# Quake4/WavPackDecoder

Hardware: AMD Instinct MI355X
Metric: Msamples/sec decoded (node) + HBM GB/s, batched 44.1kHz/16-bit stereo blocks (higher is better)
Workload: dtype int32; 1 GPU; C2: 1024-block batch, 16-bit stereo 'fast' {17,17}, joint stereo, 44.1 kHz; slices_rank0=1, blocks_rank0=1024, frames_rank0=22579200, frames_total=22579200, parallelism=file-shard x1, no collectives

## Files before the change

wavpackdecoder_amd/csrc/wv_lane.h:

```cpp
#pragma once
#include <hip/hip_runtime.h>

#include "wv_wave2.h"

namespace wvg {
namespace lane {

constexpr uint32_t ST_REDO = 1u << 15;
constexpr int RU = 32;
constexpr int GF = 8;
constexpr int NLD = 4;
constexpr int LPAIRS = 2;

__device__ __forceinline__ int32_t aw(int32_t w, int32_t s) {
    return (int32_t)(((int64_t)w * (int64_t)s + 512) >> 10);
}

template <int T, int U, bool MONO>
__device__ __forceinline__ void lp_frame(int32_t &wA, int32_t &wB, const int32_t dl, int32_t *hA, int32_t *hB, int32_t &L,
                                         int32_t &R) {
    using namespace wvf;
    static_assert(!MONO || T > 0, "mono lists have positive terms only");
    if constexpr (T == 17 || T == 18) {
        const int32_t sa = T == 17 ? sub32(mul32(2, hA[0]), hA[1]) : (sub32(mul32(3, hA[0]), hA[1]) >> 1);
// ... 579 lines not shown
            } else {
                s.zacc = lgamma(s, ring, rbase);
                if (s.zacc > 0u) {
                    s.m[0][0] = s.m[0][1] = s.m[0][2] = 0;
                    s.m[1][0] = s.m[1][1] = s.m[1][2] = 0;
                    zskip = true;
                }
            }
        }
    }
    const uint64_t zm = lmask(zskip);
    const uint64_t hzm = h0m0 | zm;
    if constexpr (HY) {
        s.slow[C] = zskip ? lhy_decay(s.slow[C]) : s.slow[C];
        if constexpr (C == 0) lhy_errlim(s, ring, !zskip);
    }
    const uint32_t lo = (uint32_t)s.win;
    uint32_t raw = (uint32_t)__builtin_ctz(~lo | 0x10000u);
    uint32_t p = raw + 1u;
    const uint64_t escm = lmask(raw >= 16u) & ~hzm;
    if (__builtin_expect(escm != 0ull, 0)) {
        if (__builtin_amdgcn_inverse_ballot_w64(escm)) {
            if (lo & 0x10000u) s.pmax = 17u;
            lskip(s, 17u);
            lrefill(s, ring, rbase);
            raw = lgamma(s, ring, rbase) + 16u;
            if (raw >= (1u << 24)) s.pmax = 17u;
            p = 0u;
        }
    }
    p = vselm(hzm, 0u, p);
    lskip(s, p);
    lrefill(s, ring, rbase);
    const uint32_t ones = vselm(hzm, 0u, addc(raw >> 1, h1m0));
    const uint64_t b0m = lmask((raw & 1u) != 0u);
    s.h1 = lbit(~hzm & b0m) ? 1u : 0u;
    s.keep = lbit(~hzm & ~b0m) ? 0u : ~0u;
    const int32_t m0 = s.m[C][0], m1 = s.m[C][1], m2 = s.m[C][2];
    const uint32_t a0 = (uint32_t)(m0 >> 4), a1 = (uint32_t)(m1 >> 4), a2 = (uint32_t)(m2 >> 4);
    const uint64_t o0 = lmask(ones == 0u), o1 = lmask(ones == 1u), o2 = lmask(ones == 2u), ob = o0 | o1;
    const uint32_t mc = vselm(o0, a0, vselm(o1, a1, a2));
    const uint32_t low1 = a0 + 1u;
    const uint32_t low2 = (ones > 2u ? ones - 2u : 0u) * (a2 + 1u) + low1 + a1 + 1u;
    const uint32_t low = vselm(o0, 0u, vselm(o1, low1, low2));
    s.m[C][0] = add32(m0, mul32((int32_t)(add3((uint32_t)m0, 128u, (uint32_t)csel<-2, 0>(o0))) >> 7, csel<-2, 5>(o0)));
    s.m[C][1] = add32(m1, mul32((int32_t)(add3((uint32_t)m1, 64u, (uint32_t)csel<-2, 0>(o1))) >> 6,
                                vselmi(o0, 0, csel<-2, 5>(o1))));
    s.m[C][2] = add32(m2, mul32((int32_t)(add3((uint32_t)m2, 32u, (uint32_t)csel<-2, 0>(o2))) >> 5,
                                vselmi(ob, 0, csel<-2, 5>(o2))));
    const uint32_t x = (uint32_t)s.win;
    uint32_t mid, used, lo_f = 0u, n_f = 1u;
    if constexpr (HY) {
        lhy_code<HY>(x, low, mc, s.el[C], mid, used, s.bad, lo_f, n_f);
        s.slack = min(s.slack, 31 - (int32_t)used);
    } else {
        const uint32_t z = (uint32_t)__builtin_clz(mc | 1u);
        const uint32_t ones_z = 0xFFFFFFFFu >> z;
        const uint32_t ex = ones_z - mc;
        const uint32_t nbt = z ^ 31u;
        const uint32_t v = x & (ones_z >> 1);
        const uint64_t bigm = lmask(v >= ex);
        const uint32_t code = vselm(bigm, 2u * v + __builtin_amdgcn_ubfe(x, nbt, 1) - ex, v);
        used = addc(nbt, bigm);
        mid = low + code;
    }
    const int32_t sg = __builtin_amdgcn_sbfe((int32_t)x, used, 1);
    lskip(s, vselm(zm, 0u, used + 1u));
    LW w;
    w.v = (int32_t)vselm(zm, 0u, mid ^ (uint32_t)sg);
    w.x = vselm(zm, 0u, x);
    w.low = vselm(zm, 0u, low);
    w.mc = vselm(zm, 0u, mc);
    w.clo = vselm(zm, 0u, mid);
    w.cn = 1u;
    if constexpr (HY == 2) {
        const bool inexact = !zskip && s.el[C] != 0;
        w.clo = inexact ? lo_f : w.clo;
        w.cn = inexact ? n_f : 1u;
    }
    if constexpr (HY) s.slow[C] = zskip ? s.slow[C] : lhy_slow(s.slow[C], mid, ring);
    lrefill(s, ring, rbase);
    return w;
}

template <int C>
__device__ __forceinline__ LW lword_fast(LState &s, const uint8_t *ring, uint32_t rbase) {
    using namespace wvf;
    const uint32_t zx = (((uint32_t)(s.m[0][0] | s.m[1][0])) & ~1u) | (s.keep + 1u) | s.h1;
    const uint32_t zrv = zx == 0u ? 1u : 0u;
    const uint32_t zdec = min(s.zacc, zrv);
    s.zacc -= zdec;
    const uint32_t zsk = min(s.zacc, zdec);
    const uint32_t lo = (uint32_t)s.win;
    const uint32_t raw = (uint32_t)__builtin_ctz(~lo | 0x10000u);
    const uint32_t keep = s.keep & (zsk - 1u);
    const uint32_t p = (raw + 1u) & keep;
    s.rare |= ((p + 15u) >> 5) | (zrv & (zdec ^ 1u));
    const uint32_t ones = ((raw >> 1) + s.h1) & keep;
    const uint32_t nh1 = raw & 1u & keep;
    s.h1 = nh1;
    s.keep = (uint32_t)__builtin_amdgcn_sbfe((int32_t)(nh1 | ~keep), 0, 1);
    s.win >>= p;
    s.nb -= (int32_t)p;
    const int32_t m0 = s.m[C][0], m1 = s.m[C][1], m2 = s.m[C][2];
    const uint32_t a0 = (uint32_t)(m0 >> 4), a1 = (uint32_t)(m1 >> 4), a2 = (uint32_t)(m2 >> 4);
    const bool o0 = ones == 0u, o1 = ones == 1u, o2 = ones == 2u, ob = ones < 2u;
    const uint32_t mc = o0 ? a0 : (o1 ? a1 : a2);
    const uint32_t low1 = a0 + 1u;
    const uint32_t low2 = __umul24(ones > 2u ? ones - 2u : 0u, a2 + 1u) + low1 + a1 + 1u;
    const uint32_t low = o0 ? 0u : (o1 ? low1 : low2);
    s.m[C][0] = mad24((add32(m0, o0 ? 126 : 128)) >> 7, o0 ? -2 : 5, m0);
    s.m[C][1] = mad24((add32(m1, o1 ? 62 : 64)) >> 6, o0 ? 0 : (o1 ? -2 : 5), m1);
    s.m[C][2] = mad24((add32(m2, o2 ? 30 : 32)) >> 5, ob ? 0 : (o2 ? -2 : 5), m2);
    const uint32_t x = (uint32_t)s.win;
    const uint32_t z = (uint32_t)__builtin_clz(mc | 1u);
    const uint32_t ones_z = 0xFFFFFFFFu >> z;
    const uint32_t ex = ones_z - mc;
    const uint32_t nbt = z ^ 31u;
    const uint32_t v = x & (ones_z >> 1);
    const bool big = v >= ex;
    const uint32_t code = big ? 2u * v + __builtin_amdgcn_ubfe(x, nbt, 1) - ex : v;
    const uint32_t used = nbt + (big ? 1u : 0u);
    const uint32_t mid = low + code;
    const int32_t sg = __builtin_amdgcn_sbfe((int32_t)x, used, 1);
    const uint32_t len = (used + 1u) & (zsk - 1u);
    s.win >>= len;
    s.nb -= (int32_t)len;
    s.slack = min(s.slack, s.nb);
    LW w;
    w.v = (int32_t)((mid ^ (uint32_t)sg) & (zsk - 1u));
    w.x = x & (zsk - 1u);
    w.low = low & (zsk - 1u);
    w.mc = mc & (zsk - 1u);
    w.clo = 0u;
    w.cn = 1u;
    lrefill(s, ring, rbase);
    return w;
}

template <bool NONNEG = true>
__device__ __forceinline__ void lmerge(LState &s, const uint8_t *ring) {
    const uint32_t mg = (uint32_t)((s.nb - 33) >> 31);
    uint32_t sh = (uint32_t)s.nb;
    if constexpr (NONNEG) __builtin_assume(sh < 64u);
    else sh &= 63u;
    s.win |= (uint64_t)(s.nxt & mg) << sh;
    s.nb = mad24((int32_t)mg, -32, s.nb);
    s.ra = ring_step(s.ra, mg);
    s.nxt = *(const uint32_t *)(ring + s.ra);
}
#ifndef WV_LANE_SPEC
#define WV_LANE_SPEC 0
#endif
template <int C, bool SPLIT, int HY = false, bool W32 = false>
__device__ __forceinline__ LW lword_nz(LState &s, const uint8_t *ring, uint32_t rbase) {
    static_assert(!HY || SPLIT, "a hybrid word's bisection bits follow a refill");
    using namespace wvf;
    constexpr bool SPEC = WV_LANE_SPEC && !SPLIT && !HY && !W32;
    const uint32_t lo = (uint32_t)s.win, hi = (uint32_t)(s.win >> 32);
    const uint32_t raw0 = SPEC ? s.r0 : (uint32_t)__builtin_ctz(~lo | 0x10000u);
    uint32_t ehi = 0u;
    if constexpr (SPEC) {
        const uint32_t sft = (uint32_t)(s.nb - 32) & 63u;
        ehi = hi | (uint32_t)((uint64_t)s.nxt << sft);
    }
    s.rmax = max(s.rmax, raw0);
    const uint32_t raw = raw0 & s.keep;
    const uint32_t ones = (raw >> 1) + s.h1;
    const uint32_t q = raw - s.keep;
    s.h1 = raw & 1u;
    s.keep = (uint32_t)__builtin_amdgcn_sbfe((int32_t)(raw | ~s.keep), 0, 1);
    if constexpr (HY && C == 0) lhy_errlim(s, ring, true);
    const int32_t m0 = s.m[C][0], m1 = s.m[C][1], m2 = s.m[C][2];
    const uint32_t a0 = (uint32_t)(m0 >> 4), a1 = (uint32_t)(m1 >> 4), a2 = (uint32_t)(m2 >> 4);
    const bool o0 = ones == 0u, o1 = ones == 1u;
    const uint32_t mc = o0 ? a0 : (o1 ? a1 : a2);
    const uint32_t l3 = (W32 ? (ones > 2u ? ones - 2u : 0u) * (a2 + 1u) : mul_u24(ones > 2u ? ones - 2u : 0u, a2 + 1u)) +
                        a1 + 1u;
    const uint32_t low = vselm(lmask(o0), 0u, add3(a0, 1u, vselm(lmask(o1), 0u, l3)));
    const uint32_t k4 = min(ones, 3u) << 2;
    const int32_t d0 = (int32_t)add3((uint32_t)m0, 128u, (uint32_t)__builtin_amdgcn_sbfe(0x000E, k4, 4)) >> 7;
    const int32_t d1 = (int32_t)add3((uint32_t)m1, 64u, (uint32_t)__builtin_amdgcn_sbfe(0x00E0, k4, 4)) >> 6;
    const int32_t d2 = (int32_t)add3((uint32_t)m2, 32u, (uint32_t)__builtin_amdgcn_sbfe(0x0E00, k4, 4)) >> 5;
    const int32_t x0 = __builtin_amdgcn_sbfe(0x555E, k4, 4), x1 = __builtin_amdgcn_sbfe(0x55E0, k4, 4);
    const int32_t x2 = __builtin_amdgcn_sbfe(0x5E00, k4, 4);
    if constexpr (W32) {
        s.m[C][0] = wvf::add32(m0, wvf::mul32(d0, x0));
        s.m[C][1] = wvf::add32(m1, wvf::mul32(d1, x1));
        s.m[C][2] = wvf::add32(m2, wvf::mul32(d2, x2));
    } else {
        s.m[C][0] = mad24(d0, x0, m0);
        s.m[C][1] = mad24(d1, x1, m1);
        s.m[C][2] = mad24(d2, x2, m2);
    }
    uint32_t x;
    if constexpr (SPLIT) {
        __builtin_assume(q < 64u);
        s.win >>= q;
        s.nb -= (int32_t)q;
        s.slack = min(s.slack, s.nb);
        lmerge<false>(s, ring);
        x = (uint32_t)s.win;
    } else {
        x = __builtin_amdgcn_alignbit(hi, lo, q);
    }
    uint32_t mid, used, lo_f = 0u, n_f = 1u;
    if constexpr (HY) {
        lhy_code<HY>(x, low, mc, s.el[C], mid, used, s.bad, lo_f, n_f);
        s.slack = min(s.slack, 31 - (int32_t)used);
    } else {
        const uint32_t z = (uint32_t)__builtin_clz(mc | 1u);
        const uint32_t ex = (0xFFFFFFFFu >> z) - mc;
        const uint32_t nbt = z ^ 31u;
        const uint32_t v = __builtin_amdgcn_ubfe(x, 0, nbt);
        const bool big = v >= ex;
        const uint32_t t = v + __builtin_amdgcn_ubfe(x, nbt, 1) - ex;
        mid = add3(low, v, big ? t : 0u);
        used = nbt + (big ? 1u : 0u);
    }
    const int32_t sg = __builtin_amdgcn_sbfe((int32_t)x, used, 1);
    const uint32_t tot = SPLIT ? used + 1u : add3(q, used, 1u);
    __builtin_assume(tot < 64u);
    if constexpr (SPEC) s.r0 = (uint32_t)__builtin_ctz(~(uint32_t)((((uint64_t)ehi << 32) | lo) >> tot) | 0x10000u);
    s.win >>= tot;
    s.nb -= (int32_t)tot;
    s.slack = min(s.slack, s.nb);
    if constexpr (!SPLIT) lmerge(s, ring);
    if constexpr (HY) s.slow[C] = lhy_slow(s.slow[C], mid, ring);
#ifdef WV_LANE_WORD_BARRIER
    __builtin_amdgcn_sched_barrier(WV_LANE_WORD_BARRIER);
#endif
    uint32_t clo = mid, cn = 1u;
    if constexpr (HY == 2) {
        clo = s.el[C] != 0 ? lo_f : mid;
        cn = s.el[C] != 0 ? n_f : 1u;
    }
    return LW{x, low, mc, (int32_t)(mid ^ (uint32_t)sg), clo, cn};
}

constexpr int RF = 24;
static_assert(RF % GF == 0, "a group's frames never wrap the frame ring");
constexpr uint32_t LSPIN = 1u << 24;

struct LShared {
    int4 rq[RF * 64];
    int2 rm[RF * 64];
    uint32_t pflag[64];
    uint32_t produced, consumed, abort;
    uint32_t hop_out[3], hop_in[3];
    uint32_t rbh[2][64];
};

__device__ __forceinline__ uint32_t rpos(const LState &s) { return s.rp + (((s.ra0 - s.ra) & RSLOT) >> 8); }

template <int HY>
__device__ __forceinline__ uint32_t pverdict(const LState &s, uint32_t u0) {
    const uint32_t r = s.bad | (s.pmax >= 17u ? 16u : 0u) | (s.slack < 0 ? 32u : 0u) | (rpos(s) >= u0 * 4u ? 64u : 0u);
    return 0x80000000u | r | ((s.bad0 ? s.bad0 : r) << 8);
}

enum { WK_CHECKED = 0, WK_FAST = 1, WK_NORUN = 2, WK_NORUN_SPLIT = 3, WK_NORUN_SPLIT32 = 4 };
template <int K, int C, int HY>
__device__ __forceinline__ LW lword_k(LState &s, const uint8_t *ring, uint32_t rb) {
    if constexpr (K == WK_NORUN) return lword_nz<C, false, false>(s, ring, rb);
    else if constexpr (K == WK_NORUN_SPLIT) return lword_nz<C, true, HY>(s, ring, rb);
    else if constexpr (K == WK_NORUN_SPLIT32) return lword_nz<C, true, HY, true>(s, ring, rb);
    else if constexpr (K == WK_FAST) return lword_fast<C>(s, ring, rb);
    else return lword<C, HY>(s, ring, rb);
}
template <int U, bool FULL, int FAST, bool MONO, int HY, bool CODES>
__device__ __forceinline__ void pframe(LState &s, const uint8_t *ring, uint32_t rb, LShared &sh, uint32_t lane,
                                       uint32_t g0, uint32_t nfr, uint32_t u0, uint32_t &pfin) {
    const uint32_t t = g0 + U;
    const uint32_t slot = (((g0 % (uint32_t)RF) + U) << 6) + lane;
    const LW w0 = lword_k<FAST, 0, HY>(s, ring, rb);
    LW w1 = {0u, 0u, 0u, 0, 0u, 1u};
    if constexpr (!MONO) w1 = lword_k<FAST, 1, HY>(s, ring, rb);
    if constexpr (CODES) {
        sh.rq[slot] = make_int4((int32_t)w0.x, (int32_t)w0.low, (int32_t)w1.x, (int32_t)w1.low);
        sh.rm[slot] = make_int2((int32_t)w0.mc, (int32_t)w1.mc);
    } else {
        sh.rm[slot] = make_int2(w0.v, w1.v);
        if constexpr (HY == 2)
            sh.rq[slot] = make_int4((int32_t)w0.clo, (int32_t)w0.cn, (int32_t)w1.clo, (int32_t)w1.cn);
    }
    if (!FULL && t + 1u == nfr) pfin = pverdict<HY>(s, u0);
}
template <bool FULL, int FAST, bool MONO, int HY, bool CODES>
__device__ __forceinline__ void pgroup(LState &s, const uint8_t *ring, uint32_t rb, LShared &sh, uint32_t lane,
                                       uint32_t g0, uint32_t nfr, uint32_t u0, uint32_t &pfin) {
    pframe<0, FULL, FAST, MONO, HY, CODES>(s, ring, rb, sh, lane, g0, nfr, u0, pfin);
    pframe<1, FULL, FAST, MONO, HY, CODES>(s, ring, rb, sh, lane, g0, nfr, u0, pfin);
    pframe<2, FULL, FAST, MONO, HY, CODES>(s, ring, rb, sh, lane, g0, nfr, u0, pfin);
    pframe<3, FULL, FAST, MONO, HY, CODES>(s, ring, rb, sh, lane, g0, nfr, u0, pfin);
    pframe<4, FULL, FAST, MONO, HY, CODES>(s, ring, rb, sh, lane, g0, nfr, u0, pfin);
    pframe<5, FULL, FAST, MONO, HY, CODES>(s, ring, rb, sh, lane, g0, nfr, u0, pfin);
    pframe<6, FULL, FAST, MONO, HY, CODES>(s, ring, rb, sh, lane, g0, nfr, u0, pfin);
    pframe<7, FULL, FAST, MONO, HY, CODES>(s, ring, rb, sh, lane, g0, nfr, u0, pfin);
}
#ifndef WV_LANE_COUNTERS
#define WV_LANE_COUNTERS 0
#endif
#define LCNT(x)                                 \
    do {                                        \
        if constexpr (WV_LANE_COUNTERS != 0) x; \
    } while (0)
struct LCount {
    uint32_t groups, bulk, norun, split, fast, checked, replay;
    uint64_t wait_consumed, wait_loads;
    uint64_t words, stage;
};
template <bool FULL, bool MONO, int HY, bool CODES>
__device__ __forceinline__ void pgroup_try(LState &s, const uint8_t *ring, uint32_t rb, LShared &sh, uint32_t lane,
                                           uint32_t g0, uint32_t nfr, uint32_t u0, uint32_t &pfin, uint32_t mm,
                                           LCount &cnt) {
    LCNT(cnt.groups++);
    const uint32_t livem = (uint32_t)((int32_t)(g0 - nfr) >> 31);
    s.slack = 0;
    constexpr uint32_t WPG = MONO ? GF : 2 * GF;
    const uint32_t notrun = (((uint32_t)(s.m[0][0] | s.m[1][0])) & ~1u) | ~s.keep | s.h1 | (s.zacc <= WPG ? 1u : 0u);
    if (lmask((notrun & livem) != 0u) == 0ull) {
#pragma unroll
        for (int u = 0; u < GF; u++) {
            const uint32_t slot = (((g0 % (uint32_t)RF) + u) << 6) + lane;
            if constexpr (CODES) sh.rq[slot] = make_int4(0, 0, 0, 0);
            if constexpr (HY == 2) sh.rq[slot] = make_int4(0, 1, 0, 1);
            sh.rm[slot] = make_int2(0, 0);
            if constexpr (HY) {
                s.slow[0] = lhy_decay(s.slow[0]);
                if constexpr (!MONO) s.slow[1] = lhy_decay(s.slow[1]);
            }
        }
        s.zacc -= WPG;
        if (!FULL && livem && nfr <= g0 + GF) pfin = pverdict<HY>(s, u0);
        LCNT(cnt.bulk++);
        return;
    }
    const uint32_t mml = mm & livem;
    const bool m26 = lmask(mml >= (1u << 26)) != 0ull;
    const uint32_t runnable = ((uint32_t)(max(s.m[0][0], s.m[1][0]) - (2 + 2 * GF)) >> 31) | min(s.zacc, 1u);
#ifndef WV_LANE_HY_PATH
#define WV_LANE_HY_PATH 0
#endif
    const bool allnr = lmask((runnable & livem) != 0u) == 0ull &&
                       !(HY && ((WV_LANE_HY_PATH == 1 && m26) || WV_LANE_HY_PATH == 2));
    if (__builtin_expect(m26 && !allnr, 0)) {
        pgroup<FULL, WK_CHECKED, MONO, HY, CODES>(s, ring, rb, sh, lane, g0, nfr, u0, pfin);
        s.bad |= s.slack < 0 ? 32u : 0u;
        LCNT(cnt.checked++);
        return;
    }
    const LState s0 = s;
    const uint32_t pfin0 = pfin;
    if (allnr) {
        s.rmax = 0u;
        if (__builtin_expect(m26, 0)) {
            pgroup<FULL, WK_NORUN_SPLIT32, MONO, HY, CODES>(s, ring, rb, sh, lane, g0, nfr, u0, pfin);
            lmerge<false>(s, ring);
            LCNT(cnt.split++);
        } else if (!HY && lmask(mml >= (1u << 17)) == 0ull) {
            if constexpr (WV_LANE_SPEC) s.r0 = (uint32_t)__builtin_ctz(~(uint32_t)s.win | 0x10000u);
            pgroup<FULL, WK_NORUN, MONO, HY, CODES>(s, ring, rb, sh, lane, g0, nfr, u0, pfin);
            LCNT(cnt.norun++);
        } else {
            pgroup<FULL, WK_NORUN_SPLIT, MONO, HY, CODES>(s, ring, rb, sh, lane, g0, nfr, u0, pfin);
            lmerge<false>(s, ring);
            LCNT(cnt.split++);
        }
        s.rare = s.rmax >> 4;
    } else if constexpr (HY) {
        s.slack = 0;
        pgroup<FULL, WK_CHECKED, MONO, HY, CODES>(s, ring, rb, sh, lane, g0, nfr, u0, pfin);
        s.bad |= s.slack < 0 ? 32u : 0u;
        LCNT(cnt.checked++);
        return;
    } else {
        s.rare = 0u;
        pgroup<FULL, WK_FAST, MONO, HY, CODES>(s, ring, rb, sh, lane, g0, nfr, u0, pfin);
        LCNT(cnt.fast++);
    }
    if (__builtin_expect(lmask(((s.rare | ((uint32_t)s.slack >> 31)) & livem) != 0u) != 0ull, 0)) {
        s = s0;
        pfin = pfin0;
        s.slack = 0;
        pgroup<FULL, WK_CHECKED, MONO, HY, CODES>(s, ring, rb, sh, lane, g0, nfr, u0, pfin);
        s.bad |= s.slack < 0 ? 32u : 0u;
        LCNT(cnt.replay++);
    }
}

struct LEnd {
    uint32_t *st;
    int32_t ml;
    bool check;
    int32_t crc;
    const uint32_t *pflag;
    uint32_t lane;
};
__device__ __forceinline__ void lane_finish(uint32_t rbad, const LEnd &e, int32_t mx, int32_t mn, uint32_t crc) {
    const uint32_t pf = e.pflag[e.lane];
    const uint32_t bad = (rbad | (pf & 0xFFu) | (mx > e.ml || mn < -e.ml ? 8u : 0u));
    uint32_t st = 0;
    if (e.check) {
        st |= ST_CRC_CHECKED;
        if ((int32_t)crc != e.crc) st |= ST_CRC_ERROR;
    }
    *e.st = bad ? (ST_REDO | (bad << 16) | (((pf >> 8) & 0xFFu) << 24)) : st;
}

__device__ __forceinline__ void st2(int32_t *p, int2 v) {
    p[0] = v.x;
    p[1] = v.y;
}

template <int HY>
__device__ __forceinline__ int32_t lfix(int32_t x, uint32_t sh, const Fixup &fx) {
    if constexpr (HY) return fixup_tail(fx, x);
    else return (int32_t)((uint32_t)x << sh);
}
__device__ __forceinline__ int32_t rdecode(uint32_t x, uint32_t low, uint32_t mc) {
    const uint32_t z = (uint32_t)__builtin_clz(mc | 1u);
    const uint32_t ex = (0xFFFFFFFFu >> z) - mc;
    const uint32_t nbt = z ^ 31u;
    const uint32_t v = __builtin_amdgcn_ubfe(x, 0, nbt);
    const bool big = v >= ex;
    const uint32_t t = v + __builtin_amdgcn_ubfe(x, nbt, 1) - ex;
    const uint32_t used = nbt + (big ? 1u : 0u);
    const int32_t sg = __builtin_amdgcn_sbfe((int32_t)x, used, 1);
    return (int32_t)(add3(low, v, big ? t : 0u) ^ (uint32_t)sg);
}
template <int U, bool MONO, bool CODES>
__device__ __forceinline__ void rin(const LShared &shr, uint32_t lane, uint32_t g0, int32_t &L, int32_t &R) {
    const uint32_t slot = (((g0 % (uint32_t)RF) + U) << 6) + lane;
    const int2 r = shr.rm[slot];
    if constexpr (CODES) {
        const int4 q = shr.rq[slot];
        L = rdecode((uint32_t)q.x, (uint32_t)q.y, (uint32_t)r.x);
        R = MONO ? 0 : rdecode((uint32_t)q.z, (uint32_t)q.w, (uint32_t)r.y);
    } else {
        L = r.x;
        R = r.y;
    }
}
template <int U, bool FULL, bool MONO, int HY>
__device__ __forceinline__ void rout(int32_t L, int32_t R, uint32_t g0, uint32_t nfr, bool joint, int32_t &mx,
                                     int32_t &mn, uint32_t &crc, uint32_t sh, int32_t *o, uint32_t rbad, const LEnd &e,
                                     bool fst, const Fixup &fx, const CWin &cw) {
    const uint32_t t = g0 + U;
    if constexpr (MONO) {
        mx = max(mx, L);
        mn = min(mn, L);
        crc = crc * 3u + (uint32_t)L;
        const int32_t v = lfix<HY>(L, sh, fx);
        const bool st = FULL ? nfr != 0u : t < nfr;
        if (st) {
            if (fst) st2(o + 2u * t, make_int2(v, v));
            else o[t] = v;
        }
        if (!FULL && t + 1u == nfr) lane_finish(rbad | (HY == 2 && (cw.used > cw.end || cw.ovf) ? 1u : 0u), e, mx, mn, crc);
        return;
    }
    if (joint) {
        R = wvf::sub32(R, L >> 1);
        L = wvf::add32(L, R);
    }
    mx = max(mx, max(L, R));
    mn = min(mn, min(L, R));
    crc = crc * 9u + (uint32_t)L * 3u + (uint32_t)R;
    int2 v;
    v.x = lfix<HY>(L, sh, fx);
    v.y = lfix<HY>(R, sh, fx);
    if (FULL) {
        if (nfr) st2(o + 2u * t, v);
    } else {
        if (t < nfr) st2(o + 2u * t, v);
        if (t + 1u == nfr) lane_finish(rbad | (HY == 2 && (cw.used > cw.end || cw.ovf) ? 1u : 0u), e, mx, mn, crc);
    }
}
template <int U, bool FULL, bool MONO, int HY, bool CODES, int... Ts>
__device__ __forceinline__ void rframe(LChain<Ts...> &ch, const LShared &shr, uint32_t lane, uint32_t g0, uint32_t nfr,
                                       bool joint, int32_t &mx, int32_t &mn, uint32_t &crc, uint32_t sh, int32_t *o,
                                       uint32_t rbad, const LEnd &e, bool fst, const Fixup &fx, CWin &cw) {
    const uint32_t t = g0 + U;
    int32_t L, R;
    rin<U, MONO, CODES>(shr, lane, g0, L, R);
    if constexpr (HY == 2) {
        const int4 q = shr.rq[(((g0 % (uint32_t)RF) + U) << 6) + lane];
        int32_t cL = 0, cR = 0;
        if (FULL || t < nfr) {
            cL = cwin_corr(cw, L, (uint32_t)q.x, (uint32_t)q.y);
            cR = cwin_corr(cw, R, (uint32_t)q.z, (uint32_t)q.w);
        }
        ch.template frame_wvc<U, MONO>(L, R, cL, cR);
        L = wvf::add32(L, cL);
        R = wvf::add32(R, cR);
    } else {
        ch.template frame<U, MONO>(L, R);
    }
    rout<U, FULL, MONO, HY>(L, R, g0, nfr, joint, mx, mn, crc, sh, o, rbad, e, fst, fx, cw);
}
template <bool FULL, bool MONO, bool CODES, int NS, int HY = 0>
__device__ __forceinline__ void rgroup_rt(RChain<NS> &ch, const LShared &shr, uint32_t lane, uint32_t g0, uint32_t nfr,
                                          bool joint, int32_t &mx, int32_t &mn, uint32_t &crc, uint32_t sh, int32_t *o,
                                          uint32_t rbad, const LEnd &e, bool fst, const Fixup &fx, const CWin &cw) {
    int32_t L[GF], R[GF];
    rin<0, MONO, CODES>(shr, lane, g0, L[0], R[0]);
    rin<1, MONO, CODES>(shr, lane, g0, L[1], R[1]);
    rin<2, MONO, CODES>(shr, lane, g0, L[2], R[2]);
    rin<3, MONO, CODES>(shr, lane, g0, L[3], R[3]);
    rin<4, MONO, CODES>(shr, lane, g0, L[4], R[4]);
    rin<5, MONO, CODES>(shr, lane, g0, L[5], R[5]);
    rin<6, MONO, CODES>(shr, lane, g0, L[6], R[6]);
    rin<7, MONO, CODES>(shr, lane, g0, L[7], R[7]);
    ch.template group<MONO>(L, R);
    rout<0, FULL, MONO, HY>(L[0], R[0], g0, nfr, joint, mx, mn, crc, sh, o, rbad, e, fst, fx, cw);
    rout<1, FULL, MONO, HY>(L[1], R[1], g0, nfr, joint, mx, mn, crc, sh, o, rbad, e, fst, fx, cw);
    rout<2, FULL, MONO, HY>(L[2], R[2], g0, nfr, joint, mx, mn, crc, sh, o, rbad, e, fst, fx, cw);
    rout<3, FULL, MONO, HY>(L[3], R[3], g0, nfr, joint, mx, mn, crc, sh, o, rbad, e, fst, fx, cw);
    rout<4, FULL, MONO, HY>(L[4], R[4], g0, nfr, joint, mx, mn, crc, sh, o, rbad, e, fst, fx, cw);
    rout<5, FULL, MONO, HY>(L[5], R[5], g0, nfr, joint, mx, mn, crc, sh, o, rbad, e, fst, fx, cw);
    rout<6, FULL, MONO, HY>(L[6], R[6], g0, nfr, joint, mx, mn, crc, sh, o, rbad, e, fst, fx, cw);
    rout<7, FULL, MONO, HY>(L[7], R[7], g0, nfr, joint, mx, mn, crc, sh, o, rbad, e, fst, fx, cw);
}

template <int HY, int... Ts>
constexpr bool lane_codes() { return !HY && (LaneRt<Ts...>::NS ? LaneRt<Ts...>::NS : (int)sizeof...(Ts)) <= 5; }

__device__ __forceinline__ uint32_t lane_shift(const BlockDesc &d) {
    int32_t sh = d.shift;
    if (d.flags & wvf::INT32_DATA)
        sh += d.int32_sent_bits ? d.int32_zeros + d.int32_sent_bits + d.int32_ones + d.int32_dups : d.int32_zeros;
    return (uint32_t)sh & 31u;
}

template <bool MONO, int HY, int... Ts>
__device__ __forceinline__ bool lane_ok(const BlockDesc &d) {
    using namespace wvf;
    if (d.kind != KIND_PCM) return false;
    if constexpr (HY == 2) {
        static_assert(!MONO, "hybrid .wvc lanes: stereo");
        if ((d.flags & (HYBRID_FLAG | HYBRID_BITRATE | INT32_DATA)) != (HYBRID_FLAG | HYBRID_BITRATE)) return false;
    } else if constexpr (HY) {
        if (!(d.flags & HYBRID_FLAG) || (d.wvx_state & 0x100)) return false;
    } else if (d.flags & (HYBRID_FLAG | FLOAT_DATA)) {
        return false;
    } else if (d.flags & INT32_DATA) {
        if (d.wvx_state & 0x100) return false;
        if (d.int32_sent_bits == 0 && d.int32_zeros == 0 && (d.int32_ones | d.int32_dups) != 0) return false;
        if (d.int32_sent_bits == 0 && d.int32_zeros != 0 && d.int32_zeros + (d.shift & 31) > 31) return false;
    }
    if (((d.flags & MONO_DATA) != 0) != MONO) return false;
    if ((d.wvc_len != 0) != (HY == 2)) return false;
    if (d.inherit || d.chain_len >= 2 || d.wvx_state || d.xfloat || d.pre_end || d.fstatus) return false;
    if constexpr (LaneRt<Ts...>::NS != 0) {
        static_assert(HY <= 1, "run-time lists: lossless or hybrid without .wvc");
        if (d.num_terms < 0 || d.num_terms > LaneRt<Ts...>::NS) return false;
        for (int i = 0; i < d.num_terms; i++) {
            const int t = d.term[i];
            if (!((t >= 1 && t <= 8) || t == 17 || t == 18 || (!MONO && t < 0 && t >= -3))) return false;
        }
        return true;
    }
    if (d.num_terms != (int32_t)sizeof...(Ts)) return false;
    constexpr int8_t terms[sizeof...(Ts) + 1] = {(int8_t)Ts..., 0};
    for (int i = 0; i < (int)sizeof...(Ts); i++)
        if (d.term[i] != terms[i]) return false;
    return true;
}

struct LBlock {
    uint32_t bi, nfr, nmax, nmin;
    bool ok, inl;
    uint32_t tw[4];
    int32_t nt;
};
template <bool MONO, int HY, int... Ts>
__device__ __forceinline__ LBlock lane_block(const BlockDesc *descs, const uint32_t *list, uint32_t n, uint32_t grp,
                                             uint32_t lane) {
    LBlock b;
    const uint32_t li = grp * 64u + lane;
    b.inl = li < n && list[li] != kLaneGap;
    b.bi = b.inl ? list[li] : 0u;
    b.ok = b.inl && lane_ok<MONO, HY, Ts...>(descs[b.bi]);
    b.tw[0] = b.tw[1] = b.tw[2] = b.tw[3] = 0u;
    b.nt = 0;
    if constexpr (LaneRt<Ts...>::NS != 0) {
        const uint64_t m = lmask(b.ok);
        if (m != 0ull) {
            const uint32_t f = (uint32_t)__builtin_ctzll(m);
            const BlockDesc &d = descs[b.bi];
            const uint32_t *tp = (const uint32_t *)d.term;
            const int32_t nt = d.num_terms;
            b.nt = __builtin_amdgcn_readlane(nt, f);
            bool same = nt == b.nt;
#pragma unroll
            for (int k = 0; k < 4; k++) {
                const uint32_t w = tp[k];
                b.tw[k] = __builtin_amdgcn_readlane(w, f);
                const int32_t nb = min(max(b.nt - 4 * k, 0), 4);
                const uint32_t bm = nb >= 4 ? ~0u : ((1u << (8 * nb)) - 1u);
                same = same && ((w ^ b.tw[k]) & bm) == 0u;
            }
            b.ok = b.ok && same;
        }
    }
    b.nfr = b.ok ? descs[b.bi].nframes : 0u;
    uint32_t nmax = b.nfr, nmin = b.nfr ? b.nfr : 0xFFFFFFFFu;
#pragma unroll
    for (int off = 32; off >= 1; off >>= 1) {
        nmax = max(nmax, (uint32_t)__shfl_xor((int)nmax, off));
        nmin = min(nmin, (uint32_t)__shfl_xor((int)nmin, off));
    }
    b.nmax = __builtin_amdgcn_readfirstlane(nmax);
    b.nmin = __builtin_amdgcn_readfirstlane(nmin);
    return b;
}

__device__ __forceinline__ bool lwait(uint32_t *ctr, uint32_t v, uint32_t *abort_flag) {
    for (uint32_t spins = 0; spins < LSPIN; spins++) {
        if (w2::uni(w2::lds_load_acq(ctr)) >= v) return true;
        if (w2::uni(w2::lds_load_acq(abort_flag))) return false;
        __builtin_amdgcn_s_sleep(1);
    }
    w2::lds_store_rel(abort_flag, 1u);
    return false;
}

template <bool MONO, int HY, int... Ts>
__device__ __forceinline__ void lane_parser(const BlockDesc *__restrict__ descs, const uint32_t *__restrict__ list,
                                            uint32_t n, const uint8_t *__restrict__ blob, LShared &sh,
                                            uint8_t *ringm, uint32_t pair, uint32_t grp, uint32_t lane,
                                            uint32_t *__restrict__ dbg) {
    using namespace wvf;
    constexpr bool CODES = lane_codes<HY, Ts...>();
    const uint64_t t_start = WV_LANE_COUNTERS ? __builtin_readcyclecounter() : 0;
    LCount cnt = {0, 0, 0, 0, 0, 0, 0, 0, 0, 0, 0};
    const LBlock lb = lane_block<MONO, HY, Ts...>(descs, list, n, grp, lane);
    const BlockDesc &d = descs[lb.bi];
    const uint32_t nfr = lb.nfr;
    const uint8_t *ring = ringm;
    const uint32_t rb = pair * RING_BYTES + lane * 4u;

    const uint64_t boff = d.bits_off;
    const uint4 *src = (const uint4 *)(blob + (boff & ~(uint64_t)15));
    const uint32_t skip = (uint32_t)(boff & 15u);
    const uint32_t e = lb.ok ? skip + d.bits_len : 0u;
    const uint32_t eu = (e + 15u) >> 4;
    const uint32_t ulast = eu > 0u ? eu - 1u : 0u;
    const uint32_t euk = lb.ok ? eu : 0xFFFFFF00u;
#pragma unroll 4
    for (uint32_t u = 0; u < (uint32_t)RU; u++) {
        uint4 v = src[min(u, ulast)];
        if (lmask(u + 1u >= euk) != 0ull) v = ff_unit(v, u, e);
        put_unit(ringm, rb, u, v);
    }
    uint32_t fu = RU;

    LState s;
    s.rp = skip >> 2;
    s.ra = rslot(s.rp) | rb;
    s.win = (uint64_t)(*(const uint32_t *)(ring + s.ra)) |
            ((uint64_t)(*(const uint32_t *)(ring + (rslot(s.rp + 1u) | rb))) << 32);
    s.win >>= (skip & 3u) * 8u;
    s.nb = 64 - (int32_t)((skip & 3u) * 8u);
    s.rp += 2u;
    s.ra = rslot(s.rp) | rb;
    s.ra0 = s.ra;
    s.nxt = *(const uint32_t *)(ring + s.ra);
    s.keep = ~0u;
    s.h1 = 0u;
    s.rare = 0u;
    s.rmax = 0u;
    s.zacc = 0u;
    s.pmax = 0u;
    s.slack = 0;
    s.bad = 0u;
    s.bad0 = 0u;
    s.nobr = (HY && !(d.flags & HYBRID_BITRATE)) ? ~0u : 0u;
    s.bal = (HY && !MONO && (d.flags & HYBRID_BALANCE) && !s.nobr) ? ~0u : 0u;
#pragma unroll
    for (int c = 0; c < 2; c++) {
#pragma unroll
        for (int k = 0; k < 3; k++) s.m[c][k] = d.median[c][k];
        s.slow[c] = HY ? d.slow_level[c] : 0;
        s.acc[c] = HY ? d.bitrate_acc[c] : 0;
        s.dlt[c] = HY ? d.bitrate_delta[c] : 0;
        s.el[c] = 0;
    }
    uint32_t pfin = 0u;
    uint32_t cpre = 0u;
    __builtin_amdgcn_s_waitcnt(0x0F70);
    for (uint32_t g0 = 0; g0 < lb.nmax; g0 += GF) {
        const uint64_t tw0 = (WV_LANE_COUNTERS && dbg) ? __builtin_readcyclecounter() : 0;
        const uint32_t need = g0 + GF > (uint32_t)RF ? g0 + GF - RF : 0u;
        if (w2::uni(cpre) < need && !lwait(&sh.consumed, need, &sh.abort)) return;
        if (WV_LANE_COUNTERS && dbg) cnt.wait_consumed += __builtin_readcyclecounter() - tw0;
        const uint32_t u00 = (uint32_t)s.m[0][0], u01 = (uint32_t)s.m[0][1], u02 = (uint32_t)s.m[0][2];
        const uint32_t u10 = (uint32_t)s.m[1][0], u11 = (uint32_t)s.m[1][1], u12 = (uint32_t)s.m[1][2];
        const uint32_t mm = MONO ? max(max(u00, u01), u02) : max(max(max(u00, u01), max(u02, u10)), max(u11, u12));
        if constexpr (!HY) s.bad |= (mm >= (1u << 29) ? 2u : 0u);
        const uint32_t u0 = fu;
        const uint32_t room = (s.rp >> 2) + (uint32_t)RU - u0;
        const uint32_t nld = room < (uint32_t)NLD ? room : (uint32_t)NLD;
        uint4 st0 = src[min(u0, ulast)], st1 = src[min(u0 + 1u, ulast)];
        uint4 st2 = src[min(u0 + 2u, ulast)], st3 = src[min(u0 + 3u, ulast)];
        fu = u0 + nld;
        const uint64_t tg0 = (WV_LANE_COUNTERS && dbg) ? __builtin_readcyclecounter() : 0;
        if (g0 + GF < lb.nmin)
            pgroup_try<true, MONO, HY, CODES>(s, ring, rb, sh, lane, g0, nfr, u0, pfin, mm, cnt);
        else
            pgroup_try<false, MONO, HY, CODES>(s, ring, rb, sh, lane, g0, nfr, u0, pfin, mm, cnt);
        if (WV_LANE_COUNTERS && dbg) cnt.words += __builtin_readcyclecounter() - tg0;
        s.rp = rpos(s);
        s.ra0 = s.ra;
        if (s.rp >= u0 * 4u) s.bad |= 64u;
        if (!s.bad0) s.bad0 = s.bad | (s.pmax >= 17u ? 16u : 0u);
        if (WV_LANE_COUNTERS && dbg) {
            const uint64_t tl0 = __builtin_readcyclecounter();
            __builtin_amdgcn_s_waitcnt(0x0F70);
            cnt.wait_loads += __builtin_readcyclecounter() - tl0;
        }
        sh.pflag[lane] = pfin;
        w2::lds_publish(&sh.produced, g0 + GF);
        cpre = __hip_atomic_load(&sh.consumed, __ATOMIC_RELAXED, __HIP_MEMORY_SCOPE_WORKGROUP);
        const uint64_t ts0 = (WV_LANE_COUNTERS && dbg) ? __builtin_readcyclecounter() : 0;
        if (lmask(u0 + (uint32_t)NLD >= euk) != 0ull) {
            st0 = ff_unit(st0, u0, e);
            st1 = ff_unit(st1, u0 + 1u, e);
            st2 = ff_unit(st2, u0 + 2u, e);
            st3 = ff_unit(st3, u0 + 3u, e);
        }
        const uint32_t dcol = RING_DUMMY + lane * 4u;
        put_unit_at(ringm, nld > 0u ? unit_addr(rb, u0) : dcol, st0);
        put_unit_at(ringm, nld > 1u ? unit_addr(rb, u0 + 1u) : dcol, st1);
        put_unit_at(ringm, nld > 2u ? unit_addr(rb, u0 + 2u) : dcol, st2);
        put_unit_at(ringm, nld > 3u ? unit_addr(rb, u0 + 3u) : dcol, st3);
        if (WV_LANE_COUNTERS && dbg) cnt.stage += __builtin_readcyclecounter() - ts0;
    }
    if (WV_LANE_COUNTERS && dbg && lane == 0u) {
        uint32_t *o = dbg + grp * 16u;
        o[0] = (uint32_t)(__builtin_readcyclecounter() - t_start);
        o[1] = cnt.groups;
        o[2] = cnt.bulk;
        o[3] = cnt.norun;
        o[4] = cnt.split;
        o[5] = cnt.fast;
        o[6] = cnt.checked;
        o[7] = cnt.replay;
        o[8] = (uint32_t)cnt.wait_consumed;
        o[9] = (uint32_t)cnt.wait_loads;
        o[10] = (uint32_t)cnt.words;
        o[11] = (uint32_t)cnt.stage;
    }
}

template <bool MONO, int HY, int... Ts>
__device__ __forceinline__ void lane_recon(const BlockDesc *__restrict__ descs, const uint32_t *__restrict__ list,
                                           uint32_t n, const uint8_t *__restrict__ blob, int32_t *__restrict__ out,
                                           uint32_t *__restrict__ status, LShared &sh, uint8_t *lds, uint32_t pair,
                                           uint32_t grp, uint32_t lane) {
    using namespace wvf;
    constexpr bool CODES = lane_codes<HY, Ts...>();
    const LBlock lb = lane_block<MONO, HY, Ts...>(descs, list, n, grp, lane);
    const BlockDesc &d = descs[lb.bi];
    const uint32_t nfr = lb.nfr;
    const bool fst = (d.flags & FALSE_STEREO) != 0;
    if (lb.inl && !lb.ok) status[lb.bi] = ST_REDO | (1u << 16);
    const bool joint = (d.flags & JOINT_STEREO) != 0;
    const uint32_t sh_ = lane_shift(d);
    const int32_t ml = d.mute_limit;
    int32_t *o = out + d.out_off;
    constexpr int NS = LaneRt<Ts...>::NS;
    typename ChainOf<Ts...>::type ch;
    if constexpr (NS != 0) ch.init(d, lb.tw, 0, lb.nt);
    else ch.init(d, 0);
    Fixup fx;
    if constexpr (HY) fixup_init(fx, d);
    CWin cw;
    if constexpr (HY == 2) cwin_init(cw, blob, lds, pair, lane, lb.ok ? d.wvc_off : 0u, lb.ok ? d.wvc_len : 0u);
    else cw = CWin{nullptr, nullptr, 0u, 0ull, 0, 0u, 0u, 0u, 0u, 0u, 0u, 0u, 0u};
    uint32_t crc = 0xFFFFFFFFu;
    int32_t mx = 0, mn = 0;
    uint32_t rbad = 0u;
    const LEnd le = {status + lb.bi, ml, d.nframes == d.block_samples, d.crc, sh.pflag, lane};
    __builtin_amdgcn_s_waitcnt(0x0F70);
    for (uint32_t g0 = 0; g0 < lb.nmax; g0 += GF) {
        if (!lwait(&sh.produced, g0 + GF, &sh.abort)) {
            if (lb.ok && nfr > g0) status[lb.bi] = ST_REDO | (128u << 16);
            return;
        }
        rbad |= ch.wbad() ? 4u : 0u;
        CStage cst;
        if constexpr (HY == 2) cst = cwin_issue(cw);
        if constexpr (NS != 0) {
            if (g0 + GF < lb.nmin)
                rgroup_rt<true, MONO, CODES, NS, HY>(ch, sh, lane, g0, nfr, joint, mx, mn, crc, sh_, o, rbad, le, fst, fx, cw);
            else
                rgroup_rt<false, MONO, CODES, NS, HY>(ch, sh, lane, g0, nfr, joint, mx, mn, crc, sh_, o, rbad, le, fst, fx, cw);
        } else if (g0 + GF < lb.nmin) {
            rframe<0, true, MONO, HY, CODES>(ch, sh, lane, g0, nfr, joint, mx, mn, crc, sh_, o, rbad, le, fst, fx, cw);
            rframe<1, true, MONO, HY, CODES>(ch, sh, lane, g0, nfr, joint, mx, mn, crc, sh_, o, rbad, le, fst, fx, cw);
            rframe<2, true, MONO, HY, CODES>(ch, sh, lane, g0, nfr, joint, mx, mn, crc, sh_, o, rbad, le, fst, fx, cw);
            rframe<3, true, MONO, HY, CODES>(ch, sh, lane, g0, nfr, joint, mx, mn, crc, sh_, o, rbad, le, fst, fx, cw);
            rframe<4, true, MONO, HY, CODES>(ch, sh, lane, g0, nfr, joint, mx, mn, crc, sh_, o, rbad, le, fst, fx, cw);
            rframe<5, true, MONO, HY, CODES>(ch, sh, lane, g0, nfr, joint, mx, mn, crc, sh_, o, rbad, le, fst, fx, cw);
            rframe<6, true, MONO, HY, CODES>(ch, sh, lane, g0, nfr, joint, mx, mn, crc, sh_, o, rbad, le, fst, fx, cw);
            rframe<7, true, MONO, HY, CODES>(ch, sh, lane, g0, nfr, joint, mx, mn, crc, sh_, o, rbad, le, fst, fx, cw);
        } else {
            rframe<0, false, MONO, HY, CODES>(ch, sh, lane, g0, nfr, joint, mx, mn, crc, sh_, o, rbad, le, fst, fx, cw);
            rframe<1, false, MONO, HY, CODES>(ch, sh, lane, g0, nfr, joint, mx, mn, crc, sh_, o, rbad, le, fst, fx, cw);
            rframe<2, false, MONO, HY, CODES>(ch, sh, lane, g0, nfr, joint, mx, mn, crc, sh_, o, rbad, le, fst, fx, cw);
            rframe<3, false, MONO, HY, CODES>(ch, sh, lane, g0, nfr, joint, mx, mn, crc, sh_, o, rbad, le, fst, fx, cw);
            rframe<4, false, MONO, HY, CODES>(ch, sh, lane, g0, nfr, joint, mx, mn, crc, sh_, o, rbad, le, fst, fx, cw);
            rframe<5, false, MONO, HY, CODES>(ch, sh, lane, g0, nfr, joint, mx, mn, crc, sh_, o, rbad, le, fst, fx, cw);
            rframe<6, false, MONO, HY, CODES>(ch, sh, lane, g0, nfr, joint, mx, mn, crc, sh_, o, rbad, le, fst, fx, cw);
            rframe<7, false, MONO, HY, CODES>(ch, sh, lane, g0, nfr, joint, mx, mn, crc, sh_, o, rbad, le, fst, fx, cw);
        }
        if constexpr (HY == 2) cwin_stage(cw, cst, lane);
        w2::lds_publish(&sh.consumed, g0 + GF);
    }
    if (lb.ok && nfr == 0u)
        status[lb.bi] = (d.block_samples == 0u) ? ST_CRC_CHECKED | ((int32_t)0xFFFFFFFFu != d.crc ? ST_CRC_ERROR : 0u) : 0u;
}

template <int NW>
struct RSplit {
#ifndef WV_RT3_RS
#define WV_RT3_RS 6
#endif
#ifndef WV_RT3_TAILW
#define WV_RT3_TAILW 1
#endif
    static constexpr int RS = NW == 2 ? 8 : WV_RT3_RS;
    static_assert(NW * RS >= MAXP, "the roles cover every list");
    __device__ __forceinline__ static void share(int32_t nt, int role, int32_t &first, int32_t &count) {
        const int32_t q = min((nt + WV_RT3_TAILW + NW - 1) / NW, (int32_t)RS);
        first = min(q * (role - 1), nt);
        count = role < NW ? min(q, nt - first) : nt - first;
    }
};
template <bool MONO>
__device__ __forceinline__ void rin2(const int2 *ring2, uint32_t lane, uint32_t g0, int32_t (&L)[GF], int32_t (&R)[GF]) {
#pragma unroll
    for (int u = 0; u < GF; u++) {
        const int2 r = ring2[(((g0 % (uint32_t)RF) + u) << 6) + lane];
        L[u] = r.x;
        R[u] = MONO ? 0 : r.y;
    }
}
template <bool MONO, int ROLE, int NW, int HY>
__device__ __forceinline__ void lane_recon_split(const BlockDesc *__restrict__ descs, const uint32_t *__restrict__ list,
                                                 uint32_t n, int32_t *__restrict__ out, uint32_t *__restrict__ status,
                                                 LShared &sh, uint32_t grp, uint32_t lane) {
    using namespace wvf;
    static_assert(ROLE >= 1 && ROLE <= NW && NW <= 3, "roles");
    const LBlock lb = lane_block<MONO, HY, LANE_RT, 16>(descs, list, n, grp, lane);
    const BlockDesc &d = descs[lb.bi];
    const uint32_t nfr = lb.nfr;
    int32_t first, count;
    RSplit<NW>::share(lb.nt, ROLE, first, count);
    RChain<RSplit<NW>::RS> ch;
    ch.init(d, lb.tw, first, count);
    int2 *const rings2 = (int2 *)sh.rq;
    static_assert(sizeof(LShared::rq) >= 2 * RF * 64 * sizeof(int2), "two hop rings in rq");
    uint32_t rbad = 0u;
    int32_t L[GF], R[GF];
    if constexpr (ROLE < NW) {
        int2 *const rout2 = rings2 + (ROLE - 1) * RF * 64;
        uint32_t cpre = 0u;
        __builtin_amdgcn_s_waitcnt(0x0F70);
        for (uint32_t g0 = 0; g0 < lb.nmax; g0 += GF) {
            if (!lwait(ROLE == 1 ? &sh.produced : &sh.hop_out[ROLE - 1], g0 + GF, &sh.abort)) return;
            const uint32_t need = g0 + GF > (uint32_t)RF ? g0 + GF - RF : 0u;
            if (w2::uni(cpre) < need && !lwait(&sh.hop_in[ROLE], need, &sh.abort)) return;
            rbad |= ch.wbad() ? 4u : 0u;
            if constexpr (ROLE == 1) {
                rin<0, MONO, false>(sh, lane, g0, L[0], R[0]);
                rin<1, MONO, false>(sh, lane, g0, L[1], R[1]);
                rin<2, MONO, false>(sh, lane, g0, L[2], R[2]);
                rin<3, MONO, false>(sh, lane, g0, L[3], R[3]);
                rin<4, MONO, false>(sh, lane, g0, L[4], R[4]);
                rin<5, MONO, false>(sh, lane, g0, L[5], R[5]);
                rin<6, MONO, false>(sh, lane, g0, L[6], R[6]);
                rin<7, MONO, false>(sh, lane, g0, L[7], R[7]);
            } else {
                rin2<MONO>(rings2 + (ROLE - 2) * RF * 64, lane, g0, L, R);
                rbad |= sh.rbh[ROLE - 2][lane];
            }
            ch.template group<MONO>(L, R);
#pragma unroll
            for (int u = 0; u < GF; u++) rout2[(((g0 % (uint32_t)RF) + u) << 6) + lane] = make_int2(L[u], R[u]);
            sh.rbh[ROLE - 1][lane] = rbad;
            w2::lds_publish(ROLE == 1 ? &sh.consumed : &sh.hop_in[ROLE - 1], g0 + GF);
            w2::lds_publish(&sh.hop_out[ROLE], g0 + GF);
            cpre = __hip_atomic_load(&sh.hop_in[ROLE], __ATOMIC_RELAXED, __HIP_MEMORY_SCOPE_WORKGROUP);
        }
    } else {
        const bool fst = (d.flags & FALSE_STEREO) != 0;
        if (lb.inl && !lb.ok) status[lb.bi] = ST_REDO | (1u << 16);
        const bool joint = (d.flags & JOINT_STEREO) != 0;
        const uint32_t sh_ = lane_shift(d);
        int32_t *o = out + d.out_off;
        Fixup fx;
        if constexpr (HY) fixup_init(fx, d);
        const CWin cw = CWin{nullptr, nullptr, 0u, 0ull, 0, 0u, 0u, 0u, 0u, 0u, 0u, 0u, 0u};
// ... 201 lines not shown
```

Measured before the change: 32330 Msamples/s.

## Add wide no-run word path and escape-aware replay before full checked replay

Adds a WIDE word variant that decodes no-split groups with per-word merge when medians are below a larger bound, used instead of the split-and-merge path. It also adds an escape-handling split word variant, used as a cheaper replay when a group overflows or sees rare long runs, before falling back to the full checked replay. A hold counter disables the wide path for a number of groups after it overflows its slack. The aim is to cut split-path overhead and expensive checked replays, at the cost of possible double replays and extra code size and register pressure.

```diff
diff --git a/wavpackdecoder_amd/csrc/wv_lane.h b/wavpackdecoder_amd/csrc/wv_lane.h
--- a/wavpackdecoder_amd/csrc/wv_lane.h
+++ b/wavpackdecoder_amd/csrc/wv_lane.h
@@ -755,11 +755,13 @@
 #ifndef WV_LANE_SPEC
 #define WV_LANE_SPEC 0
 #endif
-template <int C, bool SPLIT, int HY = false, bool W32 = false>
+template <int C, bool SPLIT, int HY = false, bool W32 = false, bool WIDE = false, bool ESC = false>
 __device__ __forceinline__ LW lword_nz(LState &s, const uint8_t *ring, uint32_t rbase) {
     static_assert(!HY || SPLIT, "a hybrid word's bisection bits follow a refill");
+    static_assert(!WIDE || (!SPLIT && !HY && !W32), "the wide word is the plain word without the promise");
+    static_assert(!ESC || (SPLIT && !HY && !W32), "the escape word is a split word");
     using namespace wvf;
-    constexpr bool SPEC = WV_LANE_SPEC && !SPLIT && !HY && !W32;
+    constexpr bool SPEC = WV_LANE_SPEC && !SPLIT && !HY && !W32 && !WIDE;
     const uint32_t lo = (uint32_t)s.win, hi = (uint32_t)(s.win >> 32);
     const uint32_t raw0 = SPEC ? s.r0 : (uint32_t)__builtin_ctz(~lo | 0x10000u);
     uint32_t ehi = 0u;
@@ -767,10 +769,23 @@
         const uint32_t sft = (uint32_t)(s.nb - 32) & 63u;
         ehi = hi | (uint32_t)((uint64_t)s.nxt << sft);
     }
-    s.rmax = max(s.rmax, raw0);
-    const uint32_t raw = raw0 & s.keep;
+    if constexpr (!ESC) s.rmax = max(s.rmax, raw0);
+    uint32_t raw = raw0 & s.keep;
+    uint32_t q = raw - s.keep;
+    if constexpr (ESC) {
+        const bool esc = raw >= 16u;
+        if (__builtin_expect(lmask(esc) != 0ull, 0)) {
+            if (esc) {
+                if (lo & 0x10000u) s.pmax = 17u;
+                lskip(s, 17u);
+                lrefill(s, ring, rbase);
+                raw = lgamma(s, ring, rbase) + 16u;
+                if (raw >= (1u << 24)) s.pmax = 17u;
+                q = 0u;
+            }
+        }
+    }
     const uint32_t ones = (raw >> 1) + s.h1;
-    const uint32_t q = raw - s.keep;
     s.h1 = raw & 1u;
     s.keep = (uint32_t)__builtin_amdgcn_sbfe((int32_t)(raw | ~s.keep), 0, 1);
     if constexpr (HY && C == 0) lhy_errlim(s, ring, true);
@@ -828,7 +843,7 @@
     s.win >>= tot;
     s.nb -= (int32_t)tot;
     s.slack = min(s.slack, s.nb);
-    if constexpr (!SPLIT) lmerge(s, ring);
+    if constexpr (!SPLIT) lmerge<!WIDE>(s, ring);
     if constexpr (HY) s.slow[C] = lhy_slow(s.slow[C], mid, ring);
 #ifdef WV_LANE_WORD_BARRIER
     __builtin_amdgcn_sched_barrier(WV_LANE_WORD_BARRIER);
@@ -862,10 +877,20 @@
     return 0x80000000u | r | ((s.bad0 ? s.bad0 : r) << 8);
 }
 
-enum { WK_CHECKED = 0, WK_FAST = 1, WK_NORUN = 2, WK_NORUN_SPLIT = 3, WK_NORUN_SPLIT32 = 4 };
+enum {
+    WK_CHECKED = 0,
+    WK_FAST = 1,
+    WK_NORUN = 2,
+    WK_NORUN_SPLIT = 3,
+    WK_NORUN_SPLIT32 = 4,
+    WK_NORUN_WIDE = 5,
+    WK_NORUN_ESC = 6
+};
 template <int K, int C, int HY>
 __device__ __forceinline__ LW lword_k(LState &s, const uint8_t *ring, uint32_t rb) {
     if constexpr (K == WK_NORUN) return lword_nz<C, false, false>(s, ring, rb);
+    else if constexpr (K == WK_NORUN_WIDE) return lword_nz<C, false, false, false, true>(s, ring, rb);
+    else if constexpr (K == WK_NORUN_ESC) return lword_nz<C, true, false, false, false, true>(s, ring, rb);
     else if constexpr (K == WK_NORUN_SPLIT) return lword_nz<C, true, HY>(s, ring, rb);
     else if constexpr (K == WK_NORUN_SPLIT32) return lword_nz<C, true, HY, true>(s, ring, rb);
     else if constexpr (K == WK_FAST) return lword_fast<C>(s, ring, rb);
@@ -912,11 +937,14 @@
     uint32_t groups, bulk, norun, split, fast, checked, replay;
     uint64_t wait_consumed, wait_loads;
     uint64_t words, stage;
+    uint32_t wide, replay_esc, held;
 };
+constexpr uint32_t WIDE_MEDIAN = 1u << 22;
+constexpr uint32_t WIDE_HOLD = 31;
 template <bool FULL, bool MONO, int HY, bool CODES>
 __device__ __forceinline__ void pgroup_try(LState &s, const uint8_t *ring, uint32_t rb, LShared &sh, uint32_t lane,
                                            uint32_t g0, uint32_t nfr, uint32_t u0, uint32_t &pfin, uint32_t mm,
-                                           LCount &cnt) {
+                                           LCount &cnt, uint32_t &whold) {
     LCNT(cnt.groups++);
     const uint32_t livem = (uint32_t)((int32_t)(g0 - nfr) >> 31);
     s.slack = 0;
@@ -955,6 +983,7 @@
     }
     const LState s0 = s;
     const uint32_t pfin0 = pfin;
+    bool wide = false, plain = false;
     if (allnr) {
         s.rmax = 0u;
         if (__builtin_expect(m26, 0)) {
@@ -963,12 +992,24 @@
             LCNT(cnt.split++);
         } else if (!HY && lmask(mml >= (1u << 17)) == 0ull) {
             if constexpr (WV_LANE_SPEC) s.r0 = (uint32_t)__builtin_ctz(~(uint32_t)s.win | 0x10000u);
+            plain = true;
             pgroup<FULL, WK_NORUN, MONO, HY, CODES>(s, ring, rb, sh, lane, g0, nfr, u0, pfin);
             LCNT(cnt.norun++);
         } else {
-            pgroup<FULL, WK_NORUN_SPLIT, MONO, HY, CODES>(s, ring, rb, sh, lane, g0, nfr, u0, pfin);
-            lmerge<false>(s, ring);
-            LCNT(cnt.split++);
+            const bool wok = !HY && lmask(mml >= WIDE_MEDIAN) == 0ull;
+            if (wok && whold == 0u) {
+                wide = plain = true;
+                pgroup<FULL, WK_NORUN_WIDE, MONO, HY, CODES>(s, ring, rb, sh, lane, g0, nfr, u0, pfin);
+                LCNT(cnt.wide++);
+            } else {
+                if (wok) {
+                    whold--;
+                    LCNT(cnt.held++);
+                }
+                pgroup<FULL, WK_NORUN_SPLIT, MONO, HY, CODES>(s, ring, rb, sh, lane, g0, nfr, u0, pfin);
+                lmerge<false>(s, ring);
+                LCNT(cnt.split++);
+            }
         }
         s.rare = s.rmax >> 4;
     } else if constexpr (HY) {
@@ -983,6 +1024,19 @@
         LCNT(cnt.fast++);
     }
     if (__builtin_expect(lmask(((s.rare | ((uint32_t)s.slack >> 31)) & livem) != 0u) != 0ull, 0)) {
+        if (wide && lmask(((uint32_t)s.slack >> 31) & livem) != 0ull) whold = WIDE_HOLD;
+        if constexpr (!HY) {
+            if (allnr && !m26 && (plain || lmask((s.rare & livem) != 0u) != 0ull)) {
+                s = s0;
+                pfin = pfin0;
+                s.slack = 0;
+                pgroup<FULL, WK_NORUN_ESC, MONO, HY, CODES>(s, ring, rb, sh, lane, g0, nfr, u0, pfin);
+                lmerge<false>(s, ring);
+                LCNT(cnt.replay_esc++);
+                const uint32_t again = (s.pmax != s0.pmax ? 1u : 0u) | ((uint32_t)s.slack >> 31);
+                if (__builtin_expect(lmask((again & livem) != 0u) == 0ull, 1)) return;
+            }
+        }
         s = s0;
         pfin = pfin0;
         s.slack = 0;
@@ -1237,7 +1291,8 @@
     using namespace wvf;
     constexpr bool CODES = lane_codes<HY, Ts...>();
     const uint64_t t_start = WV_LANE_COUNTERS ? __builtin_readcyclecounter() : 0;
-    LCount cnt = {0, 0, 0, 0, 0, 0, 0, 0, 0, 0, 0};
+    LCount cnt = {0, 0, 0, 0, 0, 0, 0, 0, 0, 0, 0, 0, 0, 0};
+    uint32_t whold = 0u;
     const LBlock lb = lane_block<MONO, HY, Ts...>(descs, list, n, grp, lane);
     const BlockDesc &d = descs[lb.bi];
     const uint32_t nfr = lb.nfr;
@@ -1310,9 +1365,9 @@
         fu = u0 + nld;
         const uint64_t tg0 = (WV_LANE_COUNTERS && dbg) ? __builtin_readcyclecounter() : 0;
         if (g0 + GF < lb.nmin)
-            pgroup_try<true, MONO, HY, CODES>(s, ring, rb, sh, lane, g0, nfr, u0, pfin, mm, cnt);
+            pgroup_try<true, MONO, HY, CODES>(s, ring, rb, sh, lane, g0, nfr, u0, pfin, mm, cnt, whold);
         else
-            pgroup_try<false, MONO, HY, CODES>(s, ring, rb, sh, lane, g0, nfr, u0, pfin, mm, cnt);
+            pgroup_try<false, MONO, HY, CODES>(s, ring, rb, sh, lane, g0, nfr, u0, pfin, mm, cnt, whold);
         if (WV_LANE_COUNTERS && dbg) cnt.words += __builtin_readcyclecounter() - tg0;
         s.rp = rpos(s);
         s.ra0 = s.ra;
@@ -1354,6 +1409,9 @@
         o[9] = (uint32_t)cnt.wait_loads;
         o[10] = (uint32_t)cnt.words;
         o[11] = (uint32_t)cnt.stage;
+        o[12] = cnt.wide;
+        o[13] = cnt.replay_esc;
+        o[14] = cnt.held;
     }
 }
 
```

After: 26690 Msamples/s. -17.5%, worse.
